# LinXueyuanStdio/LaTeX_OCR

Hardware: AMD Instinct MI355X
Metric: formula-images/sec training step (batch 64, 128x512) (higher is better)
Workload: dtype bf16

## Files before the change

### include/lxo.h

```cpp
#ifndef LXO_H
#define LXO_H
#include <stddef.h>
#include <stdint.h>
#ifdef __cplusplus
extern "C" {
#endif
#pragma GCC visibility push(default)

#define LXO_F32 0
#define LXO_BF16 1

const char* lxo_last_error(void);
#define LXO_ABI_VERSION 6
int lxo_version(void);
int lxo_shape_size(void);


int lxo_gemm_nt(int dt, int a_f32, int c_f32, int small, const void* A, const void* Bp, void* C,
                int M, int N, int K, int lda, int ldb, int ldc, const float* bias, int act,
                float alpha, int accumulate, void* stream);

int lxo_gemm_tn(int dt, int a_f32, int b_f32, const void* A, const void* B, float* C,
                int M, int I, int J, int lda, int ldb, int ldc, int nsplit, int atomic, void* stream);

// ... 54 lines not shown

int lxo_encoder_fwd(const lxo_shape* s, const float* params, const void* wpack, void* ws,
                    const uint8_t* img, void* stream);
int lxo_encoder_bwd(const lxo_shape* s, const float* params, const void* wpack, void* ws,
                    const uint8_t* img, float* grads, int last_layer, int first_layer, void* stream);
int lxo_encoder_bwd_ready(const lxo_shape* s, const float* params, const void* wpack, void* ws, const uint8_t* img, float* grads,
                          int last_layer, int first_layer, void* const* ready_events, void* stream);
int lxo_train_bwd(const lxo_shape* s, const float* params, const void* wpack, void* ws, const int32_t* formula, const uint8_t* img,
                  float* grads, void* const* ready_events, void* stream);

int lxo_set_side_stream(void* stream);
int lxo_set_encoder_side_stream(void* stream);

int lxo_decoder_train_fwd(const lxo_shape* s, const float* params, const void* wpack, void* ws,
                          const int32_t* formula, void* stream);
int lxo_ce_loss_fwd_bwd(const lxo_shape* s, void* ws, const int32_t* formula,
                        const int32_t* lengths, float inv_ntok, void* stream);
int lxo_ce_loss_fwd_bwd_dev(const lxo_shape* s, void* ws, const int32_t* formula,
                            const int32_t* lengths, const float* ntok_dev, void* stream);
int lxo_ce_loss_weighted(const lxo_shape* s, void* ws, const int32_t* formula, const int32_t* lengths,
                         const float* w_tok, const float* w_row, float inv_norm, const float* norm_dev, void* stream);
int lxo_ce_loss_smoothed(const lxo_shape* s, void* ws, const int32_t* formula, const int32_t* lengths, float eps,
                         const float* w_tok, const float* w_row, float inv_norm, const float* norm_dev, void* stream);
int lxo_mrt_weights(const float* seq_logp, const float* cost, const int32_t* group_off, int G, int rows, float alpha,
                    float* w_out, float* q_out, float* risk_out, void* stream);
#define LXO_EDIT_MAX_REF 1024
int lxo_edit_distance(const int32_t* hyp, int hyp_block, long long hyp_block_stride, long long hyp_row_stride, long long hyp_tok_stride, int T,
                      const int32_t* hyp_len, const int32_t* ref, int G, int ref_ld, const int32_t* ref_len, const int32_t* ref_of, int per_ref,
                      int pairs, int id_end, int32_t* dist_out, float* cost_out, void* stream);
#define LXO_TEXT_STATS  12
// ... 109 lines not shown
```

### latex_ocr_amd/_abi.py

```python
import ctypes
import os

c_int, c_ll, c_size, c_float, c_void = ctypes.c_int, ctypes.c_longlong, ctypes.c_size_t, ctypes.c_float, ctypes.c_void_p
P = ctypes.POINTER

LXO_F32, LXO_BF16 = 0, 1
LXO_GNORM_FLOATS = 2 + 1024
LIB_PATH = os.environ.get("LXO_LIB_PATH") or os.path.join(os.path.dirname(os.path.abspath(__file__)), "liblxo.so")


ABI_VERSION = 6
LXO_COMM_ID_BYTES = 128
LXO_I32, LXO_U8 = 2, 3
LXO_XDEC_BLOCK_BYTES, LXO_XDEC_ERR_WORD = 4096 + (384 << 10), 512
LXO_EDIT_MAX_REF = 1024
LXO_CONSENSUS_MAX_N = 64
LXO_TEXT_STATS, LXO_TEXT_CORPUS = 12, 14


class LxoShape(ctypes.Structure):
    _fields_ = [(n, c_int) for n in ("B", "H", "W", "T", "V", "C", "E", "U", "O", "D", "dtype", "beam", "max_steps")] + \
               [("keep_prob", c_float), ("dropout_seed", c_int), ("div_gamma", c_float), ("div_prob", c_float), ("div_seed", c_int),
                ("encoder_cnn", c_int), ("no_positional", c_int), ("step_kernels", c_int), ("encoder_rnn", c_int), ("deterministic", c_int), ("live_B", c_int)]

# ... 30 lines not shown
        "lxo_param_name": (ctypes.c_char_p, [c_int]),
        "lxo_param_name_for": (ctypes.c_char_p, [S, c_int]),
        "lxo_param_total": (c_ll, [S]),
        "lxo_param_info": (c_int, [S, c_int, P(c_ll), P(c_ll)]),
        "lxo_wpack_bytes": (c_size, [S]),
        "lxo_workspace_bytes": (c_size, [S]),
        "lxo_ws_region": (c_int, [S, ctypes.c_char_p, P(c_size), P(c_size)]),
        "lxo_pack_weights": (c_int, [S, c_void, c_void, c_void]),
        "lxo_encoder_fwd": (c_int, [S, c_void, c_void, c_void, c_void, c_void]),
        "lxo_encoder_bwd": (c_int, [S, c_void, c_void, c_void, c_void, c_void, c_int, c_int, c_void]),
        "lxo_encoder_bwd_ready": (c_int, [S, c_void, c_void, c_void, c_void, c_void, c_int, c_int, c_void, c_void]),
        "lxo_train_bwd": (c_int, [S, c_void, c_void, c_void, c_void, c_void, c_void, c_void, c_void]),
        "lxo_set_encoder_side_stream": (c_int, [c_void]),
        "lxo_set_side_stream": (c_int, [c_void]),
        "lxo_decoder_train_fwd": (c_int, [S, c_void, c_void, c_void, c_void, c_void]),
        "lxo_ce_loss_fwd_bwd": (c_int, [S, c_void, c_void, c_void, c_float, c_void]),
        "lxo_ce_loss_fwd_bwd_dev": (c_int, [S, c_void, c_void, c_void, c_void, c_void]),
        "lxo_ce_loss_weighted": (c_int, [S, c_void, c_void, c_void, c_void, c_void, c_float, c_void, c_void]),
        "lxo_ce_loss_smoothed": (c_int, [S, c_void, c_void, c_void, c_float, c_void, c_void, c_float, c_void, c_void]),
        "lxo_mrt_weights": (c_int, [c_void, c_void, c_void, c_int, c_int, c_float, c_void, c_void, c_void, c_void]),
        "lxo_edit_distance": (c_int, [c_void, c_int, c_ll, c_ll, c_ll, c_int, c_void, c_void, c_int, c_int, c_void, c_void, c_int, c_int, c_int, c_void, c_void, c_void]),
        "lxo_text_stats": (c_int, [c_void, c_int, c_ll, c_ll, c_ll, c_int, c_void, c_void, c_int, c_int, c_void, c_void, c_int, c_int, c_int, c_void, c_void, c_int, c_void]),
        "lxo_mrt_candidates": (c_int, [c_void, c_int, c_int, c_int, c_int, c_void, c_int, c_void, c_int, c_int, c_int, c_void, c_void, c_void, c_void, c_void, c_void]),
        "lxo_consensus": (c_int, [c_void, c_ll, c_ll, c_ll, c_int, c_int, c_int, c_int, c_void, c_int, c_void, c_void, c_void, c_void]),
        "lxo_decoder_train_bwd_part": (c_int, [S, c_void, c_void, c_void, c_void, c_void, c_int, c_void]),
        "lxo_decoder_train_bwd": (c_int, [S, c_void, c_void, c_void, c_void, c_void, c_void]),
        "lxo_global_norm_scale": (c_int, [c_ll, c_void, c_float, c_void, c_void]),
        "lxo_adam_step": (c_int, [c_ll, c_void, c_void, c_void, c_void, c_float, c_float, c_float, c_float, c_void, c_void]),
        "lxo_optimizer_step": (c_int, [c_int, c_ll, c_void, c_void, c_void, c_float, c_void, c_void]),
        "lxo_greedy_decode": (c_int, [S, c_void, c_void, c_void, c_int, c_int, c_void, P(c_int), c_void]),
# ... 34 lines not shown
            fn = getattr(lib, name)
        except AttributeError:
            missing.append(name)
            continue
        fn.restype, fn.argtypes = res, args
    lib._lxo_missing = missing
    if not missing:
        if lib.lxo_version() != ABI_VERSION or lib.lxo_shape_size() != ctypes.sizeof(LxoShape):
            raise RuntimeError("liblxo ABI mismatch: library version %d / lxo_shape %d bytes, binding version %d / %d bytes"
                               % (lib.lxo_version(), lib.lxo_shape_size(), ABI_VERSION, ctypes.sizeof(LxoShape)))
    return lib


ENTRY_POINTS = ["lxo_last_error", "lxo_version", "lxo_shape_size", "lxo_ws_region_dtype", "lxo_timing_enable", "lxo_timing_count", "lxo_timing_get", "lxo_gemm_nt", "lxo_gemm_tn", "lxo_conv3x3", "lxo_conv3x3_ex", "lxo_conv3x3_wgrad", "lxo_gemm_slab", "lxo_attention_fwd", "lxo_param_num", "lxo_param_name", "lxo_param_name_for",
                "lxo_param_total", "lxo_param_info", "lxo_wpack_bytes", "lxo_workspace_bytes", "lxo_ws_region",
                "lxo_pack_weights", "lxo_encoder_fwd", "lxo_encoder_bwd", "lxo_encoder_bwd_ready", "lxo_train_bwd", "lxo_set_side_stream", "lxo_set_encoder_side_stream", "lxo_decoder_train_fwd",
                "lxo_ce_loss_fwd_bwd", "lxo_ce_loss_fwd_bwd_dev", "lxo_ce_loss_weighted", "lxo_ce_loss_smoothed", "lxo_mrt_weights", "lxo_edit_distance", "lxo_text_stats", "lxo_mrt_candidates", "lxo_consensus", "lxo_decoder_train_bwd", "lxo_decoder_train_bwd_part", "lxo_global_norm_scale", "lxo_adam_step", "lxo_optimizer_step",
                "lxo_greedy_decode", "lxo_greedy_decode_attn", "lxo_beam_decode", "lxo_beam_decode_attn", "lxo_greedy_decode_scores", "lxo_beam_decode_scores", "lxo_score_tokens", "lxo_score_alternatives", "lxo_greedy_decode_prefix", "lxo_beam_decode_prefix", "lxo_greedy_decode_constrained", "lxo_beam_decode_constrained", "lxo_sample_decode", "lxo_sample_tokens",
                "lxo_grammar_scratch_bytes", "lxo_greedy_decode_grammar", "lxo_beam_decode_grammar", "lxo_sample_decode_grammar", "lxo_grammar_step", "lxo_decode_begin", "lxo_decode_step",
                "lxo_chain_guard", "lxo_decode_state_get", "lxo_decode_state_set", "lxo_decode_cell_step",
                "lxo_comm_unique_id", "lxo_comm_init", "lxo_comm_info", "lxo_allreduce_bucket", "lxo_comm_destroy", "lxo_comm_last_error"]

_lib = None


def load():
    global _lib
    if _lib is None:
        if not os.path.exists(LIB_PATH):
            raise RuntimeError(
                "latex_ocr_amd: %s is missing. Build it with `python -c 'import __graft_entry__ as g; g.build()'` "
# ... 15 lines not shown
```

### latex_ocr_amd/csrc/api.hip

```cpp
#include "lxo.h"
#include "gemm.h"
#include "impl.h"
#include <stdio.h>
#include <string.h>

static thread_local char g_err[256] = "";
static int fail(int code, const char* what) {
    snprintf(g_err, sizeof(g_err), "%s (code %d)", what, code);
    return code < 0 ? code : -code;
}
#define CHECK_LAUNCH(expr, what) do { int rc_ = (expr); if (rc_ != 0) return fail(rc_, what); } while (0)

extern "C" const char* lxo_last_error(void) { return g_err; }
extern "C" int lxo_version(void) { return LXO_ABI_VERSION; }
extern "C" int lxo_shape_size(void) { return (int)sizeof(lxo_shape); }

extern "C" int lxo_gemm_nt(int dt, int a_f32, int c_f32, int small, const void* A, const void* Bp, void* C,
                           int M, int N, int K, int lda, int ldb, int ldc, const float* bias, int act,
                           float alpha, int accumulate, void* stream) {
    GemmNT p; memset(&p, 0, sizeof(p));
    p.A = A; p.Bp = Bp; p.C = C; p.M = M; p.N = N; p.K = K; p.lda = lda; p.ldb = ldb; p.ldc = ldc;
    p.bias = bias; p.act = act; p.alpha = alpha; p.accumulate = accumulate; p.addend_rows = 1;
    CHECK_LAUNCH(lxo_launch_gemm_nt(dt, a_f32, c_f32, small, p, (hipStream_t)stream), "lxo_gemm_nt");
    return 0;
// ... 71 lines not shown
extern "C" int lxo_encoder_bwd_ready(const lxo_shape* s, const float* params, const void* wpack, void* ws, const uint8_t* img, float* grads,
                                     int last_layer, int first_layer, void* const* ready_events, void* stream) {
    MAKE_PLAN(P, s);
    if (last_layer > 6 || first_layer < 1 || last_layer < first_layer) return fail(-1, "lxo_encoder_bwd_ready: layer range");
    if (!ready_events) return fail(-1, "lxo_encoder_bwd_ready: null event table");
    CHECK_LAUNCH(lxo_impl_encoder_bwd(P, params, wpack, ws, img, grads, last_layer, first_layer, (hipStream_t)stream, ready_events), "lxo_encoder_bwd_ready");
    return 0;
}

#include "head_kernels.h"
extern "C" int lxo_decoder_train_fwd(const lxo_shape* s, const float* params, const void* wpack, void* ws,
                                     const int32_t* formula, void* stream) {
    MAKE_PLAN(P, s);
    if (s->T <= 0) return fail(-1, "T must be positive");
    CHECK_LAUNCH(lxo_impl_decoder_train_fwd(P, params, wpack, ws, formula, (hipStream_t)stream), "lxo_decoder_train_fwd");
    return 0;
}
extern "C" int lxo_ce_loss_fwd_bwd(const lxo_shape* s, void* ws, const int32_t* formula, const int32_t* lengths,
                                   float inv_ntok, void* stream) {
    MAKE_PLAN(P, s);
    CHECK_LAUNCH(lxo_impl_ce_loss(P, ws, formula, lengths, inv_ntok, nullptr, (hipStream_t)stream), "lxo_ce_loss_fwd_bwd");
    return 0;
}
extern "C" int lxo_ce_loss_fwd_bwd_dev(const lxo_shape* s, void* ws, const int32_t* formula, const int32_t* lengths,
                                       const float* ntok_dev, void* stream) {
    MAKE_PLAN(P, s);
    if (!ntok_dev) return fail(-1, "lxo_ce_loss_fwd_bwd_dev: null token count");
    CHECK_LAUNCH(lxo_impl_ce_loss(P, ws, formula, lengths, 0.f, ntok_dev, (hipStream_t)stream), "lxo_ce_loss_fwd_bwd_dev");
    return 0;
}
// ... 460 lines not shown
```

### latex_ocr_amd/csrc/impl.h

```cpp
#pragma once
#include "plan.h"
struct DecPrefix;
struct DecAllow;
struct DecSample;
const char* lxo_ws_name(int id);
int lxo_impl_pack_weights(const Plan& P, const float* prm, void* wp, hipStream_t st);
int lxo_impl_encoder_fwd(const Plan& P, const float* prm, const void* wp, void* ws, const uint8_t* img, hipStream_t st);
int lxo_impl_encoder_bwd(const Plan& P, const float* prm, const void* wp, void* ws, const uint8_t* img, float* grads,
                         int last_layer, int first_layer, hipStream_t st, void* const* ready = nullptr);
int lxo_impl_decoder_train_fwd(const Plan& P, const float* prm, const void* wp, void* ws, const int* formula, hipStream_t st);
int lxo_impl_ce_loss(const Plan& P, void* ws, const int* formula, const int* lengths, float inv_ntok, const float* ntok_dev, hipStream_t st,
                     const float* w_tok = nullptr, const float* w_row = nullptr, const float* smooth_eps = nullptr);
int lxo_impl_score_tokens(const Plan& P, void* ws, const int* formula, const int* lengths, float* logp_out, int* top1_out, float* seq_out, hipStream_t st);
int lxo_impl_score_alternatives(const Plan& P, void* ws, const int* formula, const int* lengths, int k, const DecAllow* allow, int* ids_out, float* logp_out,
                                int* rank_out, float* ent_out, hipStream_t st);
int lxo_impl_decoder_train_bwd(const Plan& P, const float* prm, const void* wp, void* ws, const int* formula, float* grads, int parts, hipStream_t st,
                               bool defer_join = false, void* ready = nullptr);
struct DecGrammar { const signed char* cls; int n_kinds, max_depth, budget; unsigned* scratch; int* depth; };
struct DecodeOuts { int* ids; int* parents; float* scores; float* alpha; const DecPrefix* prefix; const DecAllow* allow; const DecGrammar* grammar; };
int lxo_impl_greedy_decode(const Plan& P, const float* prm, const void* wp, void* ws, int id_end, int max_iter, const DecodeOuts& out, int* steps_out, hipStream_t st);
int lxo_impl_decode_begin(const Plan& P, const float* prm, const void* wp, void* ws, hipStream_t st);
int lxo_impl_decode_step(const Plan& P, const float* prm, const void* wp, void* ws, int id_end, int time, int* ids_out, int* parents_out, int* finished_out, int* unfinished_host, hipStream_t st);
int lxo_impl_chain_guard(const Plan& P, void* ws, const float* grads, float* scale, int have_scale, unsigned* status, hipStream_t st);
int lxo_impl_decode_state_get(const Plan& P, void* ws, int time, float* c, float* h, float* o, hipStream_t st);
int lxo_impl_decode_state_set(const Plan& P, void* ws, int time, const float* c, const float* h, const float* o, const int* ids_prev, hipStream_t st);
// ... 9 lines not shown
```

### latex_ocr_amd/csrc/model_decoder.hip

```cpp
#include "plan.h"
#include "impl.h"
#include "gemm.h"
#include "head_kernels.h"
#include "grammar.h"
#include "rstep.h"
#include "xdec.h"
#include "dimg.h"
#include "api_util.h"
#include "switches.h"
#include "timing.h"

namespace {
int nt(const Plan& P, bool a_f32, bool c_f32, bool small, const void* A, int lda, const void* Bp, int ldb, void* C, int ldc,
       int M, int N, int K, const float* bias, int act, bool accumulate, hipStream_t st) {
    GemmNT g; memset(&g, 0, sizeof(g));
    g.A = A; g.Bp = Bp; g.C = C; g.M = M; g.N = N; g.K = K; g.lda = lda; g.ldb = ldb; g.ldc = ldc;
    g.bias = bias; g.act = act; g.alpha = 1.f; g.accumulate = accumulate ? 1 : 0; g.addend_rows = 1;
    if (P.s.dtype == LXO_F32) { a_f32 = true; c_f32 = true; }
    return lxo_launch_gemm_nt(P.s.dtype, a_f32, c_f32, small, g, st);
}
int tn(const Plan& P, bool a_f32, bool b_f32, const void* A, int lda, const void* B, int ldb, float* C, int ldc,
       int M, int I, int J, hipStream_t st, DetScratch det = DetScratch{nullptr, 0}) {
    GemmTN g; memset(&g, 0, sizeof(g));
    g.A = A; g.B = B; g.C = C; g.M = M; g.I = I; g.J = J; g.lda = lda; g.ldb = ldb; g.ldc = ldc;
// ... 200 lines not shown
               P.ws<float>(ws, W_DOLOG), P.ws<float>(ws, W_G), P.ws<float>(ws, W_DHC), P.ws<float>(ws, W_DE), P.ws<float>(ws, W_DATTH),
               P.ws<float>(ws, W_DZ), P.ws<float>(ws, W_DCC), P.ws<float>(ws, W_DXH),
               P.bf ? P.ws<bf16_t>(ws, W_GB) : nullptr, P.bf ? P.ws<bf16_t>(ws, W_DZB) : nullptr};
    return w;
}

static int fwd_setup(const Train& w, const int* formula) {
    const Plan& P = w.P; void* ws = w.ws; hipStream_t st = w.st;
    const int B = P.s.B, T = P.s.T, U = P.s.U, D = P.s.D, V = P.s.V;
    RC(attention_prepare(P, w.sp, w.prm, w.wp, ws, 1, st));
    if (P.att_exp()) RC(lxo_k_att_exp(P.ws<void>(ws, W_ATT_IMG), P.ws<void>(ws, W_ATT_EXP), (long long)B * P.R * P.s.E, st));
    RC(lxo_k_embed_gather(P.s.dtype, w.prm + P.poff[P_EMB], w.prm + P.poff[P_START], formula, P.ws<void>(ws, W_EMB_IN), B, T, D, P.Dp, V, st));
    return nt(P, false, true, false, P.ws<void>(ws, W_EMB_IN), P.Dp, P.pk(w.wp, K_LSTM_XT), P.Dp, w.zx, 4 * U, T * B, 4 * U, P.Dp,
              w.prm + P.poff[P_LSTM_B], 0, false, st);
}
static int fwd_chain(const Train& w, bool* ran) {
    const Plan& P = w.P; void* ws = w.ws;
    RC(mirror_oh(P, ws, 0, P.s.B, w.st));
    XDecFwd x; memset(&x, 0, sizeof(x));
    xdec_common(x, P, w.prm, w.wp, ws);
    x.att_img = P.ws<bf16_t>(ws, W_ATT_IMG);
    x.zx = w.zx; x.gates = w.gates; x.atth = w.atth; x.alpha = w.alpha;
    x.T = P.s.T; x.Rp = P.Rp;
    x.dr = P.drop(0, 0);
    LxoTimed tm("xdec_fwd", "chain", (double)P.s.T * P.s.B * P.R * (P.s.E + P.s.C) * P.esz, w.st);
    const int rc = lxo_launch_xdec_fwd(x, P.s.U, P.s.O, P.s.C, P.s.E, w.st);
    if (rc == 0) *ran = true;
    else if (rc != -2) return rc < 0 ? rc : -rc;
    return 0;
}
static int fwd_fused_loop(const Train& w) {
    const Plan& P = w.P;
    RC(mirror_oh(P, w.ws, 0, P.s.B, w.st));
    for (int t = 0; t < P.s.T; ++t) RC(cell_step_fused(P, w.prm, w.wp, w.ws, P.s.B, 1, w.step(t), P.drop(t, 0), w.st));
    return 0;
}
static int fwd_splitk_loop(const Train& w) {
    const Plan& P = w.P;
    const int nh = w.sp.dual ? 2 : 1, hb = P.s.B / nh;
    if (w.sp.dual) RC(fork_side(w.st));
    for (int t = 0; t < P.s.T; ++t)
        for (int h = 0; h < nh; ++h)
            RC(cell_step(P, w.prm, w.wp, w.ws, h * hb, hb, 1, w.step(t, h * hb), P.drop(t, h * hb), h ? g_side : w.st));
    if (w.sp.dual) RC(join_side(w.st));
    return 0;
}
static int fwd_logits(const Train& w) {
    const Plan& P = w.P;
    const bool m = w.sp.mirrors;
    return nt(P, !m, true, false, m ? (const void*)w.step(0).recb_cur : (const void*)w.step(0).rec_cur, m ? P.RECB : P.REC, P.pk(w.wp, K_YWO_T), P.s.O,
              P.ws<float>(w.ws, W_LOGITS), P.Vp, P.s.T * P.s.B, P.s.V, P.s.O, nullptr, 0, false, w.st);
}

int lxo_impl_decoder_train_fwd(const Plan& P, const float* prm, const void* wp, void* ws, const int* formula, hipStream_t st) {
    const Train w = train_of(P, prm, wp, ws, st);
    RC(fwd_setup(w, formula));
    bool chain = false;
    if (w.sp.try_chain) RC(fwd_chain(w, &chain));
    if (P.bf && !chain) HIPRC(hipMemsetAsync(chain_block(P, ws, kChainFwd), 0, kXDecSyncBytes, st));
    if (w.sp.loop == StepPath::SplitK) RC(fwd_splitk_loop(w));
    else if (!chain) RC(fwd_fused_loop(w));
    return fwd_logits(w);
}

int lxo_impl_ce_loss(const Plan& P, void* ws, const int* formula, const int* lengths, float inv_ntok, const float* ntok_dev, hipStream_t st,
                     const float* w_tok, const float* w_row, const float* smooth_eps) {
    HIPRC(hipMemsetAsync(P.ws<float>(ws, W_LOSS), 0, 64, st));
    const CeWeights wt = {w_tok, w_row};
    const CeSmooth sm = {smooth_eps ? *smooth_eps : 0.f, smooth_eps ? *smooth_eps / (float)P.s.V : 0.f};
    RC(lxo_k_ce_loss(P.s.dtype, P.ws<float>(ws, W_LOGITS), formula, lengths, P.ws<void>(ws, W_DLOGITS), P.ws<float>(ws, W_LOSS),
                     inv_ntok, ntok_dev, chain_err(P, ws, kChainFwd), P.s.B, P.s.T, P.s.V, P.Vp,
                     DetScratch{P.ws<float>(ws, W_DET), P.wbytes[W_DET] / 4}, st,
                     (w_tok || w_row) ? &wt : nullptr, smooth_eps ? &sm : nullptr));
// ... 602 lines not shown
```

### latex_ocr_amd/csrc/xdec.h

```cpp
#pragma once
#include "lxo.h"
#include "lxo_common.h"
#include "decoder_kernels.h"
#include "lxo_debug.h"

struct XDecFwd {
    const bf16_t* Wrt; int ldrt;
    const bf16_t* Wah; int ldah;
    const bf16_t* Wow; int ldow;
    const float* beta;
    const bf16_t* att_img;
    const bf16_t* att_exp;
    const bf16_t* img;
    const float* zx;
    float* rec; bf16_t* recb;
    float* cs;
    float* gates;
    float* atth;
    float* alpha;
    float* part;
    unsigned* sync;
    int T, B, R, Rp, REC, RECB;
    Drop dr;
    unsigned long long* dbg;
};

int lxo_launch_xdec_fwd(const XDecFwd& p, int U, int O, int C, int E, hipStream_t st);

struct XDecDec {
    const bf16_t* Wrt; int ldrt; const bf16_t* Wah; int ldah; const bf16_t* Wow; int ldow;
    const bf16_t* Wyo; int ldyo;
    const float* beta;
    const bf16_t* att_exp;
    const bf16_t* img;
    const float* tx;
    float* rec; bf16_t* recb;
    float* cs;
    float* part;
    unsigned* sync;
// ... 48 lines not shown
```

### latex_ocr_amd/csrc/xdec.hip

```cpp
#include "xdec.h"
#include "drop.h"
#include "api_util.h"
#include "switches.h"

#ifdef LXO_HIPSIM
int lxo_launch_xdec_fwd(const XDecFwd&, int, int, int, int, hipStream_t) { return -2; }
int lxo_launch_xdec_bwd(const XDecBwd&, int, int, int, int, hipStream_t) { return -2; }
int lxo_launch_xdec_dec(const XDecDec&, int, int, int, int, hipStream_t) { return -2; }
extern "C" int lxo_xdec_debug(unsigned long long*) { return 0; }
extern "C" int lxo_xdec_debug_bwd(unsigned long long*) { return 0; }
#else

HIP_DYNAMIC_SHARED(char, xdec_dyn_lds)

namespace {
constexpr int XU = 512, XO = 512, XC = 512, XE = 256;
constexpr int XXH = XO + XU, XHC = XU + XC;
constexpr int OFF_H = XO, OFF_HT = XO + XU, OFF_CTX = XO + 2 * XU;
constexpr int XW = 8;
#ifndef LXO_XDEC_LLMASK
#define LXO_XDEC_LLMASK 15
#endif
constexpr int kLL = LXO_XDEC_LLMASK;
#ifndef LXO_XDEC_LLMASK_B
// ... 315 lines not shown
}

template <bool EXPD>
LXO_DEV void xdec_att_h(float (&ah)[4], const XChain& c, int ab, rsrc_t rll_ah, unsigned tag) {
    u32x4 aw[2];
    const unsigned off[2] = {(unsigned)((ab * XE + c.lane * 4) * 8), (unsigned)((ab * XE + c.lane * 4) * 8 + 16)};
    ll_wait<2>(aw, rll_ah, off, tag, c.err, c.s_dead);
#pragma unroll
    for (int j = 0; j < 4; ++j) {
        ah[j] = __uint_as_float(aw[j >> 1][(j & 1) * 2]);
        if constexpr (EXPD) ah[j] = __builtin_amdgcn_exp2f(fminf(fmaxf(ah[j] * 2.8853900817779268f, -60.f), 60.f));
    }
}

template <int ATT_U, bool EXPD>
LXO_DEV void xdec_walk(u32x4 (&xiA)[ATT_U], u32x2 (&xaA)[ATT_U], u32x4 (&xiB)[ATT_U], u32x2 (&xaB)[ATT_U], const XRole<ATT_U>& ro, int rev,
                       const float (&ah)[4], const float (&bt)[4], float& m, float& l, float (&acc)[8], float* sc, int lane) {
    const int nblk = ro.nblk;
    for (int it = 0; it < nblk; it += 2) {
        att_block<ATT_U, EXPD>(xiA, xaA, ro.XBASE(it, rev), ro.an, ah, bt, m, l, acc, sc, lane);
        __builtin_amdgcn_sched_barrier(0);
        att_load<ATT_U>(xiA, xaA, ro.imq, ro.aiq, (it + 2 < nblk) ? ro.XBASE(it + 2, rev) : ro.XBASE(0, rev ^ 1), ro.anq, lane);
        __builtin_amdgcn_sched_barrier(0);
        if (it + 1 < nblk) {
            att_block<ATT_U, EXPD>(xiB, xaB, ro.XBASE(it + 1, rev), ro.an, ah, bt, m, l, acc, sc, lane);
            __builtin_amdgcn_sched_barrier(0);
            att_load<ATT_U>(xiB, xaB, ro.imq, ro.aiq, (it + 3 < nblk) ? ro.XBASE(it + 3, rev) : ro.XBASE(1, rev ^ 1), ro.anq, lane);
            __builtin_amdgcn_sched_barrier(0);
        }
    }
}

template <int NQ, bool PP>
LXO_DEV void xdec_p3_publish(float m, float l, const float (&acc)[8], const XChain& c, int ab, int aq, int t, float* part, float* wred, float (*redc)[XC]) {
// ... 89 lines not shown
                for (int q = 0; q < QG; ++q) pc[si][q] = l2_load16(rpart, (unsigned)((((gsm * SPG + si) * NQ + cb + q) * PST + c4) * 4));
        }
        if (wave == 0) {
            const unsigned o = (unsigned)((min(tid, NB * NQ - 1) * PST + XC) * 4);
            st_m = l2_load4(rpart, o); st_l = l2_load4(rpart, o + 4);
        }
    }
    if (wave == 0) {
        float mm = st_l > 0.f ? st_m : -3.0e38f;
#pragma unroll
        for (int o = NQ / 2; o > 0; o >>= 1) mm = fmaxf(mm, __shfl_xor(mm, o));
        const float w = st_l > 0.f ? __expf(st_m - mm) : 0.f;
        float ll = st_l * w;
#pragma unroll
        for (int o = NQ / 2; o > 0; o >>= 1) ll += __shfl_xor(ll, o);
        const float inv = 1.0f / ll;
        if (tid < NB * NQ) {
            (&wgt[0][0])[tid] = w * inv;
            if constexpr (SM) { if ((tid & (NQ - 1)) == 0) { smax[tid / NQ] = mm; sinv[tid / NQ] = inv; } }
        }
    }
    __syncthreads();
    if (gsm < NG) {
#pragma unroll
        for (int si = 0; si < SPG; ++si) {
            const int sidx = gsm * SPG + si;
            float v[4] = {0.f, 0.f, 0.f, 0.f};
#pragma unroll
            for (int q0 = 0; q0 < CPG; q0 += QG) {
#pragma unroll
                for (int q = 0; q < QG; ++q) {
// ... 75 lines not shown
#define XSTAMP(step, i) do { if (dbg && tid == 0) dbg[(step) * 16 + (i)] = wall_clock64(); } while (0)

template <int NB, int ATT_U, bool EXPD>
__global__ __launch_bounds__(512) void xdec_fwd_kernel(XDecFwd p) {
    constexpr int NQ = 32 / NB;
    constexpr bool PP = (kLL & 4) != 0;
    __shared__ __attribute__((aligned(16))) float redbuf[XW * 8 * 64];
    float (*red)[8][64] = reinterpret_cast<float (*)[8][64]>(redbuf);
    float (*redc)[XC] = reinterpret_cast<float (*)[XC]>(redbuf);
    __shared__ u32x4 wahs[XW][2][64];
    __shared__ __attribute__((aligned(16))) bf16_t actx[16][XC + 8];
    __shared__ float sc[SCMAX];
    __shared__ float cst[8][16];
    __shared__ float wgt[NB][NQ], smax[NB], sinv[NB];
    __shared__ float wred[2 * XW];
    __shared__ int s_rank, s_dead;

    if constexpr (NB >= 2) asm volatile("" ::: "v254");
    XChain c = xchain_ticket(p.sync, NB, &s_rank, &s_dead);
    const int tid = c.tid, lane = c.lane, wave = c.wave, r16 = c.r16, g4 = c.g4;
    for (int i = tid; i < 16 * (XC + 8); i += 512) (&actx[0][0])[i] = 0;
    __syncthreads();
    if (!xchain_rank(c, &s_rank)) return;
    const int rank = c.rank, b0 = c.b0, u0 = rank * 16;
    unsigned* xsync = c.xsync; unsigned* err = c.err;
    const int B = p.B, T = p.T;

    u32x4 wrt0[4], wow[4];
    u32x4* wl = reinterpret_cast<u32x4*>(xdec_dyn_lds) + (wave * 12) * 64 + lane;
    float bt[4];
    xdec_resident<EXPD>(p, c, wrt0, wl, wahs, wow, bt);
    if (tid < NB * 16) cst[tid >> 4][tid & 15] = p.cs[(long long)(b0 + (tid >> 4)) * XU + u0 + (tid & 15)];

    const XRole<ATT_U> ro = xdec_role<NB, ATT_U>(c, p.R, p.img, EXPD ? p.att_exp : p.att_img);
    Drop dr = p.dr;
    unsigned ph = 0;
    u32x4 xiA[ATT_U], xiB[ATT_U]; u32x2 xaA[ATT_U], xaB[ATT_U];
    auto prefetch = [&](int ts) {
        att_load<ATT_U>(xiA, xaA, ro.imq, ro.aiq, ro.XBASE(0, ts & 1), ro.anq, lane);
        att_load<ATT_U>(xiB, xaB, ro.imq, ro.aiq, ro.XBASE(1, ts & 1), ro.anq, lane);
    };
    prefetch(0);

    float pzn[4];
    {
        const int er = min(tid >> 4, NB - 1);
        const float* zr = p.zx + (long long)(b0 + er) * 4 * XU + u0 + (tid & 15);
#pragma unroll
        for (int q = 0; q < 4; ++q) pzn[q] = zr[q * XU];
// ... 60 lines not shown
        if (kLL & 1) __syncthreads();
        else xbar(xsync, rank, ++ph, err, &s_dead);
        XSTAMP(t, 2);
        xdec_p2<NB, (kLL & 1) != 0, true>(p, c, sp, sn, t, rll_ht, ll_ah, red, wahs);
        if (kPF == 2 && t > 0) prefetch(t);
        XSTAMP(t, 3);
        if (!(kLL & 2)) xbar(xsync, rank, ++ph, err, &s_dead);
        XSTAMP(t, 4);
        {
            {
                const int er = min(tid >> 4, NB - 1);
                const float* zr = p.zx + ((long long)min(t + 1, T - 1) * B + b0 + er) * 4 * XU + u0 + (tid & 15);
#pragma unroll
                for (int q = 0; q < 4; ++q) pzn[q] = zr[q * XU];
            }
            float ah[4];
            xdec_att_h<EXPD>(ah, c, ro.ab, rll_ah, (unsigned)(t + 1));
            float m = -3.0e38f, l = 0.f, acc[8];
#pragma unroll
            for (int e = 0; e < 8; ++e) acc[e] = 0.f;
            const int rev = t & 1;
            if constexpr (kPF == 0) xdec_walk<ATT_U, EXPD>(xiA, xaA, xiB, xaB, ro, rev, ah, bt, m, l, acc, sc, lane);
            else {
                const int nblk = ro.nblk, an = ro.an, anq = ro.anq;
                int it = 0;
                for (; it + 3 < nblk; it += 2) {
                    att_block<ATT_U, EXPD>(xiA, xaA, ro.XBASE(it, rev), an, ah, bt, m, l, acc, sc, lane);
                    __builtin_amdgcn_sched_barrier(0);
                    att_load<ATT_U>(xiA, xaA, ro.imq, ro.aiq, ro.XBASE(it + 2, rev), anq, lane);
                    __builtin_amdgcn_sched_barrier(0);
                    att_block<ATT_U, EXPD>(xiB, xaB, ro.XBASE(it + 1, rev), an, ah, bt, m, l, acc, sc, lane);
                    __builtin_amdgcn_sched_barrier(0);
                    att_load<ATT_U>(xiB, xaB, ro.imq, ro.aiq, ro.XBASE(it + 3, rev), anq, lane);
                    __builtin_amdgcn_sched_barrier(0);
                }
                const int rem = nblk - it;
                if (rem >= 1) att_block<ATT_U, EXPD>(xiA, xaA, ro.XBASE(it, rev), an, ah, bt, m, l, acc, sc, lane);
                if (rem == 3) { __builtin_amdgcn_sched_barrier(0); att_load<ATT_U>(xiA, xaA, ro.imq, ro.aiq, ro.XBASE(it + 2, rev), anq, lane); __builtin_amdgcn_sched_barrier(0); }
                if (rem >= 2) att_block<ATT_U, EXPD>(xiB, xaB, ro.XBASE(it + 1, rev), an, ah, bt, m, l, acc, sc, lane);
                if (rem == 3) att_block<ATT_U, EXPD>(xiA, xaA, ro.XBASE(it + 2, rev), an, ah, bt, m, l, acc, sc, lane);
            }
            xdec_p3_publish<NQ, PP>(m, l, acc, c, ro.ab, ro.aq, t, p.part, wred, redc);
        }
        XSTAMP(t, 5);
        if constexpr (!PP) xbar(xsync, rank, ++ph, err, &s_dead);
        XSTAMP(t, 6);
        {
            u32x4 a[4];
            xdec_o_fetch(a, p, c, sn);
            xdec_p4_merge<NB, PP, true>(p, c, sn, t, wgt, smax, sinv, redc, actx, dbg ? dbg + t * 16 + 12 : nullptr);
            if (kPF == 3) prefetch(t + 1);
            {
                const float mm = smax[ro.as], inv = sinv[ro.as];
                float* al = p.alpha + (sp + ro.ab) * p.Rp + ro.ar0;
                for (int r = tid; r < ro.an; r += 512) al[r] = __expf(sc[r] - mm) * inv;
            }
            __syncthreads();
            xdec_o_proj<NB, 16>(a, p, c, sn, t, &dr, wow, actx, red, ll_o);
        }
        XSTAMP(t, 7);
        if (kLL & 8) __syncthreads();
        else xbar(xsync, rank, ++ph, err, &s_dead);
        XSTAMP(t, 8);
    }
}

template <auto KERNEL, class P>
int xdec_launch(const P& p, hipStream_t st) {
    constexpr int DYN = XW * 12 * 64 * 16;
    static bool attr_done = false;
// ... 234 lines not shown
                rr[OFF_H + u] = h; rr[OFF_HT + u] = h;
                const bf16_t htb = f2bf(h);
                rb[OFF_H + u] = htb; rb[OFF_HT + u] = htb;
                const unsigned mine = (unsigned)htb, other = (unsigned)__shfl_xor((int)mine, 1);
                if (!(eu & 1)) { const u32x2 wv = {mine | (other << 16), (unsigned)(t + 1)}; *reinterpret_cast<u32x2*>(ll_ht + ((bb * 256 + (u >> 1)) * 2)) = wv; }
            }
        }
        __syncthreads();
        xdec_p2<NB, true, false>(p, c, sp, sn, t, rll_ht, ll_ah, red, wahs);
        {
            float ah[4];
            xdec_att_h<true>(ah, c, ro.ab, rll_ah, (unsigned)(t + 1));
            float m = -3.0e38f, l = 0.f, acc[8];
#pragma unroll
            for (int e = 0; e < 8; ++e) acc[e] = 0.f;
            xdec_walk<ATT_U, true>(xiA, xaA, xiB, xaB, ro, tg & 1, ah, bt, m, l, acc, nullptr, lane);
            xdec_p3_publish<NQ, PP>(m, l, acc, c, ro.ab, ro.aq, t, p.part, wred, redc);
        }
        if constexpr (!PP) xbar(xsync, rank, ++ph, err, &s_dead);
#ifdef LXO_TEST_DEC_FAULT
        if (tg == 21 && xcc == 3u && tid == 0) { s_dead = 1; *reinterpret_cast<volatile unsigned*>(err) = 9u; }
#endif
        {
            u32x4 a[4];
            xdec_o_fetch(a, p, c, sn);
            xdec_p4_merge<NB, PP, false>(p, c, sn, t, wgt, nullptr, nullptr, redc, actx, nullptr);
            __syncthreads();
            xdec_o_proj<NB, 8>(a, p, c, sn, t, nullptr, wow, actx, red, ll_o);
        }
        __syncthreads();
    }
// ... 481 lines not shown
```

### latex_ocr_amd/engine.py

```python
import ctypes
import math
import os
from collections import OrderedDict, namedtuple

import numpy as np
import torch

from . import _abi
from .model import params as PP


Alternatives = namedtuple("Alternatives", ["ids", "logp", "rank", "entropy"])


def _p(t):
    return ctypes.c_void_p(t.data_ptr()) if t is not None else ctypes.c_void_p(0)


XDEC_BLOCK_BYTES = _abi.LXO_XDEC_BLOCK_BYTES
XDEC_STATUS_WORDS = _abi.LXO_XDEC_ERR_WORD + 1


def _chain_words(w):
    return bool(w[32:_abi.LXO_XDEC_ERR_WORD:64].any()), int(w[_abi.LXO_XDEC_ERR_WORD])
# ... 153 lines not shown
        if not ring or ring[0]["host"].numel() < n:
            cap = max(64, n)
            ring = [{"host": torch.empty(cap, dtype=torch.int32).pin_memory(), "dev": torch.empty(cap, dtype=torch.int32, device=self.device), "ev": None}
                    for _ in range(4)]
            self._len_ring, self._len_i = ring, 0
        slot = ring[self._len_i % len(ring)]
        self._len_i += 1
        if slot["ev"] is not None:
            slot["ev"].synchronize()
        slot["host"][:n].numpy()[:] = a
        slot["dev"][:n].copy_(slot["host"][:n], non_blocking=True)
        slot["ev"] = torch.cuda.Event()
        slot["ev"].record(torch.cuda.current_stream(self.device))
        return slot["dev"][:n]

    def forward(self, img, formula, dropout=None, phase_hook=None, before_decoder=None):
        B, H, W = int(img.shape[0]), int(img.shape[1]), int(img.shape[2])
        T = int(formula.shape[1])
        self.live_B = B
        drop_on = dropout is not None and 0.0 < float(dropout[0]) < 1.0
        Bp = B if drop_on else self._train_chain_batch(B, H, W)
        if Bp != B:
            if isinstance(formula, torch.Tensor):
                cache = self.__dict__.setdefault("_pad_rows", {})
                idx = cache.get((Bp, B, formula.device))
                if idx is None:
                    idx = cache[(Bp, B, formula.device)] = (torch.arange(Bp, device=formula.device) % B)
                formula = formula.index_select(0, idx)
            else:
                formula = np.ascontiguousarray(np.asarray(formula)[np.arange(Bp) % B])
        self.ensure(Bp, H, W, T)
        self.shape.live_B = B if Bp != B else 0
        B = Bp
        if dropout is not None and 0.0 < float(dropout[0]) < 1.0:
            self.shape.keep_prob = float(dropout[0])
            self.shape.dropout_seed = int(dropout[1]) & 0x7FFFFFFF
        self._img = self._to_dev(img, torch.uint8)
        self._formula = self._to_dev(formula, torch.int32)
        st = self._stream()
        self._bind_side()
        self._ck(self.lib.lxo_encoder_fwd(self.sref(), _p(self.params), _p(self.wpack), _p(self.ws), _p(self._img), st), "encoder_fwd")
        if phase_hook:
            phase_hook("encoder_fwd")
        if before_decoder is not None:
            torch.cuda.current_stream(self.device).wait_event(before_decoder)
        self._ck(self.lib.lxo_decoder_train_fwd(self.sref(), _p(self.params), _p(self.wpack), _p(self.ws), _p(self._formula), st),
                 "decoder_train_fwd")
        if (not self._xdec_checked and self.dtype == _abi.LXO_BF16 and self.step_kernels == 0 and self.device.type == "cuda"
                and (B, H, W) not in self._nochain_shapes):
            if self._check_chain():
                self._ck(self.lib.lxo_decoder_train_fwd(self.sref(), _p(self.params), _p(self.wpack), _p(self.ws), _p(self._formula), st),
                         "decoder_train_fwd")

    def chain_status(self, backward=False):
        o = XDEC_BLOCK_BYTES // 4 if backward else 0
        return _chain_words(self.region("xdec_sync", "i32")[o:o + XDEC_STATUS_WORDS].cpu().numpy())

    def _check_chain(self, backward=False):
        sfx = "_bwd" if backward else ""
        used, err = self.chain_status(backward)
        setattr(self, "chain_used" + sfx, used and not err)
        if used or err:
            setattr(self, "_xdec%s_checked" % sfx, True)
        else:
            getattr(self, "_nochain_shapes" + sfx).add((self.shape.B, self.shape.H, self.shape.W))
        if err:
            self._chain_fallback("backward" if backward else "forward", err)
# ... 100 lines not shown
        return eps

    def _weights_dev(self, w, dead):
        if isinstance(w, torch.Tensor):
            w = w.to(device=self.device, dtype=torch.float32).contiguous()
            if dead > 0:
                w = torch.cat([w, torch.zeros((dead,) + tuple(w.shape[1:]), dtype=torch.float32, device=self.device)])
            return w
        if dead > 0:
            w = np.concatenate([w, np.zeros((dead,) + w.shape[1:], np.float32)])
        t = torch.from_numpy(np.ascontiguousarray(w, dtype=np.float32))
        if self.device.type != "cuda":
            return t
        return t.pin_memory().to(self.device, non_blocking=True)

    def loss(self, lengths, inv_ntok=None, ntok_dev=None, ntok_event=None, weights=None, row_weights=None, _padded=False, label_smoothing=0.0):
        eps = self._check_smoothing("loss", label_smoothing)
        if weights is None and row_weights is None:
            self._bind_lengths(lengths)
            wt = wr = None
        else:
            live = int(getattr(self, "live_B", self.shape.B))
            dead = int(self.shape.B) - live
            if not _padded:
                weights, row_weights = self._check_weights("loss", weights, row_weights, live, int(self.shape.T))
                weights = self._weights_dev(weights, dead) if weights is not None else None
                row_weights = self._weights_dev(row_weights, dead) if row_weights is not None else None
            if lengths is not None:
                self._bind_lengths(lengths)
            wt, wr = self._loss_weights = (weights, row_weights)
        if ntok_dev is not None:
            if ntok_event is not None:
                torch.cuda.current_stream(self.device).wait_event(ntok_event)
            self._ntok_dev = ntok_dev
# ... 141 lines not shown
        if norm is not None and not (math.isfinite(float(norm)) and float(norm) != 0.0):
            raise ValueError("train_step: norm must be a finite non-zero number, got %r" % (norm,))
        wkw = dict(weights=weights, row_weights=row_weights) if weighted else {}
        if eps > 0.0:
            wkw["label_smoothing"] = eps
        drop = None
        if dropout is not None and 0.0 < float(dropout) < 1.0:
            self.drop_step = getattr(self, "drop_step", 0) + 1
            world, rank = (dist.world, dist.rank) if dist is not None else (1, 0)
            drop = (float(dropout), dropout_seed if dropout_seed is not None else self.drop_step * world + rank)
        n_local = int(np.asarray(lengths).sum()) if not isinstance(lengths, torch.Tensor) else int(lengths.sum().item())
        if self._health_ring is not None and dist is None:
            self._chain_health_poll()
        if dist is not None and norm is None:
            ntok, ev = dist.sum_count_async(n_local)
            self.forward(img, formula, dropout=drop, before_decoder=ev)
            stats = self.loss(lengths, ntok_dev=ntok, ntok_event=ev, **wkw)
        else:
            self.forward(img, formula, dropout=drop)
            stats = self.loss(lengths, 1.0 / (float(n_local) if norm is None else float(norm)), **wkw)
        self.backward(comm=dist.reduce_range_fn(self.grads) if dist is not None else None)
        if dist is not None:
            dist.finish()
        self.optimizer_step(lr, clip, guard=True, dp=dist is not None)
        if not sync_loss:
            return None
        if dist is not None:
            s = stats.clone()
            dist.all_reduce(s)
            s = s.cpu().numpy()
        else:
            s = stats.cpu().numpy()
        if (self._health_ring is not None and self._chain_health_poll(wait=True) and getattr(self, "_last_dropped_seq", -1) == self._health_i
                and dist is None and not getattr(self, "_redoing", False)):
            self._redoing = True
# ... 285 lines not shown
        if k == 0 and allowed is not None:
            raise ValueError("score: allowed= constrains the alternatives only and needs alternatives > 0")
        if k != 0 and not 1 <= k <= min(16, self.n_tok):
            raise ValueError("score: alternatives must lie in 1 .. min(16, V = %d), got %d" % (self.n_tok, k))
        al = self._allow_host(allowed, B, None, 1) if allowed is not None else None
        parts = [self._score_piece(img[i:i + 64], f[i:i + 64], ln[i:i + 64], return_top1, k,
                                   al if al is None or al.shape[0] == 1 else al[i:i + 64]) for i in range(0, B, 64)]
        logp, seq = np.concatenate([p[0] for p in parts]), np.concatenate([p[2] for p in parts])
        out = (logp, np.concatenate([p[1] for p in parts]), seq) if return_top1 else (logp, seq)
        if k:
            out += (Alternatives(*[np.concatenate([p[3][j] for p in parts]) for j in range(4)]),)
        return out

    def _score_piece(self, img, formula, lengths, top1_on, k=0, al=None):
        while True:
            self.forward(img, formula)
            B, T = int(self.shape.B), int(self.shape.T)
            live, n = int(self.live_B), B * T
            ln = np.zeros(B, np.int32)
            ln[:live] = lengths
            ln_dev = self._lengths_dev(ln)
            chain = self._chains_possible()
            na = 2 * n + B
            ns = na + (2 * n * k + 2 * n if k else 0)
            buf = torch.empty(ns + (XDEC_STATUS_WORDS if chain else 0), dtype=torch.int32, device=self.device)
            logp, top1, seq = buf[:n].view(torch.float32), buf[n:2 * n] if top1_on else None, buf[2 * n:2 * n + B].view(torch.float32)
            self._ck(self.lib.lxo_score_tokens(self.sref(), _p(self.ws), _p(self._formula), _p(ln_dev), _p(logp), _p(top1), _p(seq),
                                               self._stream()), "score_tokens")
            if k:
                alw = self._allow_args(al, live, B) if al is not None else (None, 0)
                self._ck(self.lib.lxo_score_alternatives(self.sref(), _p(self.ws), _p(self._formula), _p(ln_dev), k, _p(alw[0]), alw[1],
                                                         _p(buf[na:na + n * k]), _p(buf[na + n * k:na + 2 * n * k].view(torch.float32)),
                                                         _p(buf[na + 2 * n * k:na + 2 * n * k + n]), _p(buf[na + 2 * n * k + n:ns].view(torch.float32)),
                                                         self._stream()), "score_alternatives")
            if chain:
                buf[ns:].copy_(self.region("xdec_sync", "i32")[:XDEC_STATUS_WORDS])
# ... 424 lines not shown
```

Measured before the change: 8922.

## Skip decoder attention walk for timesteps past each sequence's length

Passes per-row target lengths into the chained decoder forward kernel so the attention block walk is skipped for padded timesteps. Alpha for those steps is written as zero and the softmax normaliser is guarded against a zero sum. Training and scoring now bind lengths before the forward pass. This cuts attention work on padding. Hidden states for padded steps are still computed but with a zero context, which changes values only at masked positions. Rows in a workgroup may diverge in length, so the saving depends on the length distribution.

```diff
diff --git a/include/lxo.h b/include/lxo.h
--- a/include/lxo.h
+++ b/include/lxo.h
@@ -92,6 +92,8 @@
 
 int lxo_decoder_train_fwd(const lxo_shape* s, const float* params, const void* wpack, void* ws,
                           const int32_t* formula, void* stream);
+int lxo_decoder_train_fwd_live(const lxo_shape* s, const float* params, const void* wpack, void* ws,
+                               const int32_t* formula, const int32_t* lengths, void* stream);
 int lxo_ce_loss_fwd_bwd(const lxo_shape* s, void* ws, const int32_t* formula,
                         const int32_t* lengths, float inv_ntok, void* stream);
 int lxo_ce_loss_fwd_bwd_dev(const lxo_shape* s, void* ws, const int32_t* formula,
diff --git a/latex_ocr_amd/_abi.py b/latex_ocr_amd/_abi.py
--- a/latex_ocr_amd/_abi.py
+++ b/latex_ocr_amd/_abi.py
@@ -68,6 +68,7 @@
         "lxo_set_encoder_side_stream": (c_int, [c_void]),
         "lxo_set_side_stream": (c_int, [c_void]),
         "lxo_decoder_train_fwd": (c_int, [S, c_void, c_void, c_void, c_void, c_void]),
+        "lxo_decoder_train_fwd_live": (c_int, [S, c_void, c_void, c_void, c_void, c_void, c_void]),
         "lxo_ce_loss_fwd_bwd": (c_int, [S, c_void, c_void, c_void, c_float, c_void]),
         "lxo_ce_loss_fwd_bwd_dev": (c_int, [S, c_void, c_void, c_void, c_void, c_void]),
         "lxo_ce_loss_weighted": (c_int, [S, c_void, c_void, c_void, c_void, c_void, c_float, c_void, c_void]),
@@ -132,7 +133,7 @@
 
 ENTRY_POINTS = ["lxo_last_error", "lxo_version", "lxo_shape_size", "lxo_ws_region_dtype", "lxo_timing_enable", "lxo_timing_count", "lxo_timing_get", "lxo_gemm_nt", "lxo_gemm_tn", "lxo_conv3x3", "lxo_conv3x3_ex", "lxo_conv3x3_wgrad", "lxo_gemm_slab", "lxo_attention_fwd", "lxo_param_num", "lxo_param_name", "lxo_param_name_for",
                 "lxo_param_total", "lxo_param_info", "lxo_wpack_bytes", "lxo_workspace_bytes", "lxo_ws_region",
-                "lxo_pack_weights", "lxo_encoder_fwd", "lxo_encoder_bwd", "lxo_encoder_bwd_ready", "lxo_train_bwd", "lxo_set_side_stream", "lxo_set_encoder_side_stream", "lxo_decoder_train_fwd",
+                "lxo_pack_weights", "lxo_encoder_fwd", "lxo_encoder_bwd", "lxo_encoder_bwd_ready", "lxo_train_bwd", "lxo_set_side_stream", "lxo_set_encoder_side_stream", "lxo_decoder_train_fwd", "lxo_decoder_train_fwd_live",
                 "lxo_ce_loss_fwd_bwd", "lxo_ce_loss_fwd_bwd_dev", "lxo_ce_loss_weighted", "lxo_ce_loss_smoothed", "lxo_mrt_weights", "lxo_edit_distance", "lxo_text_stats", "lxo_mrt_candidates", "lxo_consensus", "lxo_decoder_train_bwd", "lxo_decoder_train_bwd_part", "lxo_global_norm_scale", "lxo_adam_step", "lxo_optimizer_step",
                 "lxo_greedy_decode", "lxo_greedy_decode_attn", "lxo_beam_decode", "lxo_beam_decode_attn", "lxo_greedy_decode_scores", "lxo_beam_decode_scores", "lxo_score_tokens", "lxo_score_alternatives", "lxo_greedy_decode_prefix", "lxo_beam_decode_prefix", "lxo_greedy_decode_constrained", "lxo_beam_decode_constrained", "lxo_sample_decode", "lxo_sample_tokens",
                 "lxo_grammar_scratch_bytes", "lxo_greedy_decode_grammar", "lxo_beam_decode_grammar", "lxo_sample_decode_grammar", "lxo_grammar_step", "lxo_decode_begin", "lxo_decode_step",
diff --git a/latex_ocr_amd/csrc/api.hip b/latex_ocr_amd/csrc/api.hip
--- a/latex_ocr_amd/csrc/api.hip
+++ b/latex_ocr_amd/csrc/api.hip
@@ -109,6 +109,13 @@
     MAKE_PLAN(P, s);
     if (s->T <= 0) return fail(-1, "T must be positive");
     CHECK_LAUNCH(lxo_impl_decoder_train_fwd(P, params, wpack, ws, formula, (hipStream_t)stream), "lxo_decoder_train_fwd");
+    return 0;
+}
+extern "C" int lxo_decoder_train_fwd_live(const lxo_shape* s, const float* params, const void* wpack, void* ws,
+                                          const int32_t* formula, const int32_t* lengths, void* stream) {
+    MAKE_PLAN(P, s);
+    if (s->T <= 0) return fail(-1, "T must be positive");
+    CHECK_LAUNCH(lxo_impl_decoder_train_fwd(P, params, wpack, ws, formula, (hipStream_t)stream, lengths), "lxo_decoder_train_fwd_live");
     return 0;
 }
 extern "C" int lxo_ce_loss_fwd_bwd(const lxo_shape* s, void* ws, const int32_t* formula, const int32_t* lengths,
diff --git a/latex_ocr_amd/csrc/impl.h b/latex_ocr_amd/csrc/impl.h
--- a/latex_ocr_amd/csrc/impl.h
+++ b/latex_ocr_amd/csrc/impl.h
@@ -8,7 +8,7 @@
 int lxo_impl_encoder_fwd(const Plan& P, const float* prm, const void* wp, void* ws, const uint8_t* img, hipStream_t st);
 int lxo_impl_encoder_bwd(const Plan& P, const float* prm, const void* wp, void* ws, const uint8_t* img, float* grads,
                          int last_layer, int first_layer, hipStream_t st, void* const* ready = nullptr);
-int lxo_impl_decoder_train_fwd(const Plan& P, const float* prm, const void* wp, void* ws, const int* formula, hipStream_t st);
+int lxo_impl_decoder_train_fwd(const Plan& P, const float* prm, const void* wp, void* ws, const int* formula, hipStream_t st, const int* lengths = nullptr);
 int lxo_impl_ce_loss(const Plan& P, void* ws, const int* formula, const int* lengths, float inv_ntok, const float* ntok_dev, hipStream_t st,
                      const float* w_tok = nullptr, const float* w_row = nullptr, const float* smooth_eps = nullptr);
 int lxo_impl_score_tokens(const Plan& P, void* ws, const int* formula, const int* lengths, float* logp_out, int* top1_out, float* seq_out, hipStream_t st);
diff --git a/latex_ocr_amd/csrc/model_decoder.hip b/latex_ocr_amd/csrc/model_decoder.hip
--- a/latex_ocr_amd/csrc/model_decoder.hip
+++ b/latex_ocr_amd/csrc/model_decoder.hip
@@ -238,7 +238,7 @@
     return nt(P, false, true, false, P.ws<void>(ws, W_EMB_IN), P.Dp, P.pk(w.wp, K_LSTM_XT), P.Dp, w.zx, 4 * U, T * B, 4 * U, P.Dp,
               w.prm + P.poff[P_LSTM_B], 0, false, st);
 }
-static int fwd_chain(const Train& w, bool* ran) {
+static int fwd_chain(const Train& w, const int* lengths, bool* ran) {
     const Plan& P = w.P; void* ws = w.ws;
     RC(mirror_oh(P, ws, 0, P.s.B, w.st));
     XDecFwd x; memset(&x, 0, sizeof(x));
@@ -247,6 +247,7 @@
     x.zx = w.zx; x.gates = w.gates; x.atth = w.atth; x.alpha = w.alpha;
     x.T = P.s.T; x.Rp = P.Rp;
     x.dr = P.drop(0, 0);
+    x.lengths = lengths;
     LxoTimed tm("xdec_fwd", "chain", (double)P.s.T * P.s.B * P.R * (P.s.E + P.s.C) * P.esz, w.st);
     const int rc = lxo_launch_xdec_fwd(x, P.s.U, P.s.O, P.s.C, P.s.E, w.st);
     if (rc == 0) *ran = true;
@@ -276,11 +277,11 @@
               P.ws<float>(w.ws, W_LOGITS), P.Vp, P.s.T * P.s.B, P.s.V, P.s.O, nullptr, 0, false, w.st);
 }
 
-int lxo_impl_decoder_train_fwd(const Plan& P, const float* prm, const void* wp, void* ws, const int* formula, hipStream_t st) {
+int lxo_impl_decoder_train_fwd(const Plan& P, const float* prm, const void* wp, void* ws, const int* formula, hipStream_t st, const int* lengths) {
     const Train w = train_of(P, prm, wp, ws, st);
     RC(fwd_setup(w, formula));
     bool chain = false;
-    if (w.sp.try_chain) RC(fwd_chain(w, &chain));
+    if (w.sp.try_chain) RC(fwd_chain(w, lengths, &chain));
     if (P.bf && !chain) HIPRC(hipMemsetAsync(chain_block(P, ws, kChainFwd), 0, kXDecSyncBytes, st));
     if (w.sp.loop == StepPath::SplitK) RC(fwd_splitk_loop(w));
     else if (!chain) RC(fwd_fused_loop(w));
diff --git a/latex_ocr_amd/csrc/xdec.h b/latex_ocr_amd/csrc/xdec.h
--- a/latex_ocr_amd/csrc/xdec.h
+++ b/latex_ocr_amd/csrc/xdec.h
@@ -23,6 +23,7 @@
     int T, B, R, Rp, REC, RECB;
     Drop dr;
     unsigned long long* dbg;
+    const int* lengths;
 };
 
 int lxo_launch_xdec_fwd(const XDecFwd& p, int U, int O, int C, int E, hipStream_t st);
diff --git a/latex_ocr_amd/csrc/xdec.hip b/latex_ocr_amd/csrc/xdec.hip
--- a/latex_ocr_amd/csrc/xdec.hip
+++ b/latex_ocr_amd/csrc/xdec.hip
@@ -353,10 +353,10 @@
 }
 
 template <int ATT_U, bool EXPD>
-LXO_DEV void xdec_walk(u32x4 (&xiA)[ATT_U], u32x2 (&xaA)[ATT_U], u32x4 (&xiB)[ATT_U], u32x2 (&xaB)[ATT_U], const XRole<ATT_U>& ro, int rev,
+LXO_DEV void xdec_walk(u32x4 (&xiA)[ATT_U], u32x2 (&xaA)[ATT_U], u32x4 (&xiB)[ATT_U], u32x2 (&xaB)[ATT_U], const XRole<ATT_U>& ro, int nwalk, int rev,
                        const float (&ah)[4], const float (&bt)[4], float& m, float& l, float (&acc)[8], float* sc, int lane) {
     const int nblk = ro.nblk;
-    for (int it = 0; it < nblk; it += 2) {
+    for (int it = 0; it < nwalk; it += 2) {
         att_block<ATT_U, EXPD>(xiA, xaA, ro.XBASE(it, rev), ro.an, ah, bt, m, l, acc, sc, lane);
         __builtin_amdgcn_sched_barrier(0);
         att_load<ATT_U>(xiA, xaA, ro.imq, ro.aiq, (it + 2 < nblk) ? ro.XBASE(it + 2, rev) : ro.XBASE(0, rev ^ 1), ro.anq, lane);
@@ -476,7 +476,8 @@
         float ll = st_l * w;
 #pragma unroll
         for (int o = NQ / 2; o > 0; o >>= 1) ll += __shfl_xor(ll, o);
-        const float inv = 1.0f / ll;
+        float inv = 1.0f / ll;
+        if constexpr (SM) inv = ll > 0.f ? inv : 0.f;
         if (tid < NB * NQ) {
             (&wgt[0][0])[tid] = w * inv;
             if constexpr (SM) { if ((tid & (NQ - 1)) == 0) { smax[tid / NQ] = mm; sinv[tid / NQ] = inv; } }
@@ -582,7 +583,7 @@
     __shared__ float cst[8][16];
     __shared__ float wgt[NB][NQ], smax[NB], sinv[NB];
     __shared__ float wred[2 * XW];
-    __shared__ int s_rank, s_dead;
+    __shared__ int s_rank, s_dead, s_alen;
 
     if constexpr (NB >= 2) asm volatile("" ::: "v254");
     XChain c = xchain_ticket(p.sync, NB, &s_rank, &s_dead);
@@ -601,6 +602,7 @@
     if (tid < NB * 16) cst[tid >> 4][tid & 15] = p.cs[(long long)(b0 + (tid >> 4)) * XU + u0 + (tid & 15)];
 
     const XRole<ATT_U> ro = xdec_role<NB, ATT_U>(c, p.R, p.img, EXPD ? p.att_exp : p.att_img);
+    if (tid == 0) s_alen = p.lengths ? p.lengths[ro.ab] : T;
     Drop dr = p.dr;
     unsigned ph = 0;
     u32x4 xiA[ATT_U], xiB[ATT_U]; u32x2 xaA[ATT_U], xaB[ATT_U];
@@ -691,15 +693,17 @@
 #pragma unroll
                 for (int q = 0; q < 4; ++q) pzn[q] = zr[q * XU];
             }
+            const int alen_v = s_alen;
             float ah[4];
             xdec_att_h<EXPD>(ah, c, ro.ab, rll_ah, (unsigned)(t + 1));
+            const bool live = t < __builtin_amdgcn_readfirstlane(alen_v);
             float m = -3.0e38f, l = 0.f, acc[8];
 #pragma unroll
             for (int e = 0; e < 8; ++e) acc[e] = 0.f;
             const int rev = t & 1;
-            if constexpr (kPF == 0) xdec_walk<ATT_U, EXPD>(xiA, xaA, xiB, xaB, ro, rev, ah, bt, m, l, acc, sc, lane);
+            if constexpr (kPF == 0) xdec_walk<ATT_U, EXPD>(xiA, xaA, xiB, xaB, ro, live ? ro.nblk : 0, rev, ah, bt, m, l, acc, sc, lane);
             else {
-                const int nblk = ro.nblk, an = ro.an, anq = ro.anq;
+                const int nblk = live ? ro.nblk : 0, an = ro.an, anq = ro.anq;
                 int it = 0;
                 for (; it + 3 < nblk; it += 2) {
                     att_block<ATT_U, EXPD>(xiA, xaA, ro.XBASE(it, rev), an, ah, bt, m, l, acc, sc, lane);
@@ -730,7 +734,8 @@
             {
                 const float mm = smax[ro.as], inv = sinv[ro.as];
                 float* al = p.alpha + (sp + ro.ab) * p.Rp + ro.ar0;
-                for (int r = tid; r < ro.an; r += 512) al[r] = __expf(sc[r] - mm) * inv;
+                const int alen_a = s_alen;
+                for (int r = tid; r < ro.an; r += 512) { const float a = __expf(sc[r] - mm) * inv; al[r] = t < alen_a ? a : 0.f; }
             }
             __syncthreads();
             xdec_o_proj<NB, 16>(a, p, c, sn, t, &dr, wow, actx, red, ll_o);
@@ -995,7 +1000,7 @@
             float m = -3.0e38f, l = 0.f, acc[8];
 #pragma unroll
             for (int e = 0; e < 8; ++e) acc[e] = 0.f;
-            xdec_walk<ATT_U, true>(xiA, xaA, xiB, xaB, ro, tg & 1, ah, bt, m, l, acc, nullptr, lane);
+            xdec_walk<ATT_U, true>(xiA, xaA, xiB, xaB, ro, ro.nblk, tg & 1, ah, bt, m, l, acc, nullptr, lane);
             xdec_p3_publish<NQ, PP>(m, l, acc, c, ro.ab, ro.aq, t, p.part, wred, redc);
         }
         if constexpr (!PP) xbar(xsync, rank, ++ph, err, &s_dead);
diff --git a/latex_ocr_amd/engine.py b/latex_ocr_amd/engine.py
--- a/latex_ocr_amd/engine.py
+++ b/latex_ocr_amd/engine.py
@@ -191,7 +191,7 @@
         slot["ev"].record(torch.cuda.current_stream(self.device))
         return slot["dev"][:n]
 
-    def forward(self, img, formula, dropout=None, phase_hook=None, before_decoder=None):
+    def forward(self, img, formula, dropout=None, phase_hook=None, before_decoder=None, lengths=None):
         B, H, W = int(img.shape[0]), int(img.shape[1]), int(img.shape[2])
         T = int(formula.shape[1])
         self.live_B = B
@@ -214,6 +214,8 @@
             self.shape.dropout_seed = int(dropout[1]) & 0x7FFFFFFF
         self._img = self._to_dev(img, torch.uint8)
         self._formula = self._to_dev(formula, torch.int32)
+        if lengths is not None:
+            self._bind_lengths(lengths)
         st = self._stream()
         self._bind_side()
         self._ck(self.lib.lxo_encoder_fwd(self.sref(), _p(self.params), _p(self.wpack), _p(self.ws), _p(self._img), st), "encoder_fwd")
@@ -221,13 +223,19 @@
             phase_hook("encoder_fwd")
         if before_decoder is not None:
             torch.cuda.current_stream(self.device).wait_event(before_decoder)
-        self._ck(self.lib.lxo_decoder_train_fwd(self.sref(), _p(self.params), _p(self.wpack), _p(self.ws), _p(self._formula), st),
-                 "decoder_train_fwd")
+        self._decoder_fwd(st, lengths is not None)
         if (not self._xdec_checked and self.dtype == _abi.LXO_BF16 and self.step_kernels == 0 and self.device.type == "cuda"
                 and (B, H, W) not in self._nochain_shapes):
             if self._check_chain():
-                self._ck(self.lib.lxo_decoder_train_fwd(self.sref(), _p(self.params), _p(self.wpack), _p(self.ws), _p(self._formula), st),
-                         "decoder_train_fwd")
+                self._decoder_fwd(st, lengths is not None)
+
+    def _decoder_fwd(self, st, live):
+        if live:
+            self._ck(self.lib.lxo_decoder_train_fwd_live(self.sref(), _p(self.params), _p(self.wpack), _p(self.ws), _p(self._formula),
+                                                         _p(self._lengths), st), "decoder_train_fwd_live")
+        else:
+            self._ck(self.lib.lxo_decoder_train_fwd(self.sref(), _p(self.params), _p(self.wpack), _p(self.ws), _p(self._formula), st),
+                     "decoder_train_fwd")
 
     def chain_status(self, backward=False):
         o = XDEC_BLOCK_BYTES // 4 if backward else 0
@@ -358,10 +366,14 @@
             return t
         return t.pin_memory().to(self.device, non_blocking=True)
 
-    def loss(self, lengths, inv_ntok=None, ntok_dev=None, ntok_event=None, weights=None, row_weights=None, _padded=False, label_smoothing=0.0):
+    def loss(self, lengths, inv_ntok=None, ntok_dev=None, ntok_event=None, weights=None, row_weights=None, _padded=False, label_smoothing=0.0,
+             _bound=False):
         eps = self._check_smoothing("loss", label_smoothing)
+        if _bound:
+            lengths = None
         if weights is None and row_weights is None:
-            self._bind_lengths(lengths)
+            if lengths is not None:
+                self._bind_lengths(lengths)
             wt = wr = None
         else:
             live = int(getattr(self, "live_B", self.shape.B))
@@ -533,11 +545,11 @@
             self._chain_health_poll()
         if dist is not None and norm is None:
             ntok, ev = dist.sum_count_async(n_local)
-            self.forward(img, formula, dropout=drop, before_decoder=ev)
-            stats = self.loss(lengths, ntok_dev=ntok, ntok_event=ev, **wkw)
+            self.forward(img, formula, dropout=drop, before_decoder=ev, lengths=lengths)
+            stats = self.loss(lengths, ntok_dev=ntok, ntok_event=ev, _bound=True, **wkw)
         else:
-            self.forward(img, formula, dropout=drop)
-            stats = self.loss(lengths, 1.0 / (float(n_local) if norm is None else float(norm)), **wkw)
+            self.forward(img, formula, dropout=drop, lengths=lengths)
+            stats = self.loss(lengths, 1.0 / (float(n_local) if norm is None else float(norm)), _bound=True, **wkw)
         self.backward(comm=dist.reduce_range_fn(self.grads) if dist is not None else None)
         if dist is not None:
             dist.finish()
@@ -853,12 +865,10 @@
 
     def _score_piece(self, img, formula, lengths, top1_on, k=0, al=None):
         while True:
-            self.forward(img, formula)
+            self.forward(img, formula, lengths=np.asarray(lengths, dtype=np.int32).reshape(-1))
             B, T = int(self.shape.B), int(self.shape.T)
             live, n = int(self.live_B), B * T
-            ln = np.zeros(B, np.int32)
-            ln[:live] = lengths
-            ln_dev = self._lengths_dev(ln)
+            ln_dev = self._lengths
             chain = self._chains_possible()
             na = 2 * n + B
             ns = na + (2 * n * k + 2 * n if k else 0)
```

Result: faster. 9155, median of 6 (+2.6%).
